# westlake-repl/Adapter4Rec

Measured on NVIDIA B200. Metric: train user-sequences/s (SASRec + BERT-base LoRA r=8 adapter-tuning step: fwd+bwd+allreduce+Adam), higher is better.
Workload: dtype bf16

## Files before the change

adapter4rec_b200/csrc/a4r_common.cuh:

```cuda
#pragma once
#include <cuda.h>
#include <cuda_bf16.h>
#include <cuda_runtime.h>
#include <stdint.h>
#include <stdio.h>

#include "../../include/adapter4rec.h"

int a4r_set_error(int code, const char* fmt, ...);

#define A4R_CHECK_ARG(cond, ...)                                   \
  do {                                                              \
    if (!(cond)) return a4r_set_error(A4R_EINVAL, __VA_ARGS__);     \
  } while (0)

#define A4R_CUDA_OK(expr)                                                                  \
  do {                                                                                      \
    cudaError_t _e = (expr);                                                                \
    if (_e != cudaSuccess)                                                                  \
      return a4r_set_error(A4R_ECUDA, "%s failed: %s (%s:%d)", #expr, cudaGetErrorString(_e), \
                           __FILE__, __LINE__);                                             \
  } while (0)

#define A4R_LAUNCH_OK()                                                                   \
  do {                                                                                     \
    cudaError_t _e = cudaGetLastError();                                                   \
    if (_e != cudaSuccess)                                                                 \
      return a4r_set_error(A4R_ECUDA, "kernel launch failed: %s (%s:%d)",                  \
                           cudaGetErrorString(_e), __FILE__, __LINE__);                    \
  } while (0)

int a4r_num_sms();
void a4r_count_launch(int n);

int a4r_make_tmap_bf16(CUtensorMap* m, const void* base, int64_t rows, int64_t cols, int64_t ld, int box_rows);

static inline bool a4r_aligned16(const void* p) { return (reinterpret_cast<uintptr_t>(p) & 15u) == 0; }

#ifdef __CUDACC__

#define A4R_DEVICE __device__ __forceinline__

A4R_DEVICE uint32_t smem_u32(const void* p) { return static_cast<uint32_t>(__cvta_generic_to_shared(p)); }

A4R_DEVICE float warp_sum(float v) {
#pragma unroll
  for (int o = 16; o > 0; o >>= 1) v += __shfl_xor_sync(0xffffffffu, v, o);
  return v;
}
A4R_DEVICE float warp_max(float v) {
#pragma unroll
  for (int o = 16; o > 0; o >>= 1) v = fmaxf(v, __shfl_xor_sync(0xffffffffu, v, o));
  return v;
}

A4R_DEVICE float gelu_erf(float x) { return 0.5f * x * (1.0f + erff(x * 0.70710678118654752440f)); }
A4R_DEVICE float gelu_erf_grad(float x) {
  const float cdf = 0.5f * (1.0f + erff(x * 0.70710678118654752440f));
  const float pdf = 0.39894228040143267794f * __expf(-0.5f * x * x);
  return cdf + x * pdf;
}

A4R_DEVICE float ex2_approx(float x) {
  float r;
  asm("ex2.approx.ftz.f32 %0, %1;" : "=f"(r) : "f"(x));
  return r;
}
A4R_DEVICE float tanh_approx(float x) {
  float r;
  asm("tanh.approx.f32 %0, %1;" : "=f"(r) : "f"(x));
  return r;
}
constexpr float kGeluC0 = 0.797507884f, kGeluC1 = 0.0370056460f, kGeluC2 = -3.51516783e-4f;
A4R_DEVICE float gelu_cdf(float x) {
  const float x2 = fminf(x * x, 64.0f);
  const float u = x * fmaf(fmaf(x2, kGeluC2, kGeluC1), x2, kGeluC0);
  return fmaf(0.5f, tanh_approx(u), 0.5f);
}
A4R_DEVICE float gelu_fast(float x) { return x * gelu_cdf(x); }
A4R_DEVICE float gelu_grad_fast(float x) {
  const float e = ex2_approx(-0.72134752044448170368f * x * x);
  return fmaf(x * 0.39894228040143267794f, e, gelu_cdf(x));
}
A4R_DEVICE float2 splat2(float c) { return make_float2(c, c); }
A4R_DEVICE float2 gelu_cdf2(float2 x) {
  float2 x2 = __fmul2_rn(x, x);
  x2 = make_float2(fminf(x2.x, 64.0f), fminf(x2.y, 64.0f));
  float2 q = __ffma2_rn(x2, splat2(kGeluC2), splat2(kGeluC1));
// ... 368 lines not shown
```

adapter4rec_b200/csrc/api.cu:

```cuda
#include <stdarg.h>
#include <atomic>

#include "a4r_common.cuh"

namespace {
thread_local char g_err[512] = {0};
std::atomic<int64_t> g_launches{0};
}

int a4r_set_error(int code, const char* fmt, ...) {
  va_list ap;
  va_start(ap, fmt);
  vsnprintf(g_err, sizeof(g_err), fmt, ap);
  va_end(ap);
  return code;
}

void a4r_count_launch(int n) { g_launches.fetch_add(n, std::memory_order_relaxed); }

int a4r_num_sms() {
  static int sms = 0;
  if (sms == 0) {
    int dev = 0;
    if (cudaGetDevice(&dev) != cudaSuccess) return 148;
    if (cudaDeviceGetAttribute(&sms, cudaDevAttrMultiProcessorCount, dev) != cudaSuccess || sms <= 0) sms = 148;
  }
  return sms;
}

namespace {
typedef CUresult (*PFN_encodeTiled)(CUtensorMap*, CUtensorMapDataType, cuuint32_t, void*, const cuuint64_t*,
                                    const cuuint64_t*, const cuuint32_t*, const cuuint32_t*, CUtensorMapInterleave,
                                    CUtensorMapSwizzle, CUtensorMapL2promotion, CUtensorMapFloatOOBfill);
PFN_encodeTiled encode_fn() {
  static PFN_encodeTiled fn = nullptr;
  if (fn == nullptr) {
    void* p = nullptr;
    cudaDriverEntryPointQueryResult q;
    if (cudaGetDriverEntryPoint("cuTensorMapEncodeTiled", &p, cudaEnableDefault, &q) == cudaSuccess &&
        q == cudaDriverEntryPointSuccess)
      fn = reinterpret_cast<PFN_encodeTiled>(p);
  }
  return fn;
}
}

int a4r_make_tmap_bf16(CUtensorMap* m, const void* base, int64_t rows, int64_t cols, int64_t ld, int box_rows) {
  PFN_encodeTiled fn = encode_fn();
  if (fn == nullptr) return a4r_set_error(A4R_ECUDA, "cuTensorMapEncodeTiled entry point not found");
  cuuint64_t dims[2] = {static_cast<cuuint64_t>(cols), static_cast<cuuint64_t>(rows)};
  cuuint64_t strides[1] = {static_cast<cuuint64_t>(ld) * 2};
  cuuint32_t box[2] = {64u, static_cast<cuuint32_t>(box_rows)};
  cuuint32_t estr[2] = {1, 1};
  CUresult r = fn(m, CU_TENSOR_MAP_DATA_TYPE_BFLOAT16, 2, const_cast<void*>(base), dims, strides, box, estr,
                  CU_TENSOR_MAP_INTERLEAVE_NONE, CU_TENSOR_MAP_SWIZZLE_128B, CU_TENSOR_MAP_L2_PROMOTION_L2_256B,
                  CU_TENSOR_MAP_FLOAT_OOB_FILL_NONE);
  if (r != CUDA_SUCCESS)
    return a4r_set_error(A4R_ECUDA, "cuTensorMapEncodeTiled failed (%d) rows=%lld cols=%lld ld=%lld", (int)r,
                         (long long)rows, (long long)cols, (long long)ld);
  return A4R_OK;
}

extern "C" int a4r_version(void) { return 100;  }

extern "C" const char* a4r_last_error_string(void) { return g_err; }

extern "C" int64_t a4r_launch_count(void) { return g_launches.load(std::memory_order_relaxed); }

extern "C" int a4r_device_check(void) {
  static int cached_dev = -1;
  static int cached_rc = A4R_OK;
  int dev = 0;
  cudaError_t e = cudaGetDevice(&dev);
  if (e != cudaSuccess) return a4r_set_error(A4R_ECUDA, "cudaGetDevice failed: %s", cudaGetErrorString(e));
  if (dev == cached_dev) {
    if (cached_rc != A4R_OK) a4r_set_error(cached_rc, "device %d is not compute capability 10.x (sm_100a only)", dev);
    return cached_rc;
  }
  int major = 0;
  e = cudaDeviceGetAttribute(&major, cudaDevAttrComputeCapabilityMajor, dev);
  if (e != cudaSuccess) return a4r_set_error(A4R_ECUDA, "cudaDeviceGetAttribute failed: %s", cudaGetErrorString(e));
  cached_dev = dev;
  cached_rc = (major == 10) ? A4R_OK : A4R_EARCH;
  if (cached_rc != A4R_OK)
    return a4r_set_error(A4R_EARCH, "device %d has compute capability %d.x; this library is sm_100a only", dev, major);
  return A4R_OK;
}
```

adapter4rec_b200/functional.py:

```python
import torch

from . import ops

BF16 = torch.bfloat16


PARAM_EPOCH = [0]


def bump_param_epoch():
    PARAM_EPOCH[0] += 1


class WeightCache:

    def __init__(self):
        self.key = None
        self.master = None
        self.w = None
        self.wt = None

    def get(self, weight, need_t=False):
        key = (weight.data_ptr(), weight._version, weight.device, PARAM_EPOCH[0] if weight.requires_grad else -1)
        if key != self.key:
# ... 355 lines not shown
    first = torch.full((uh.numel(),), N, dtype=torch.int64, device=rows.device)
    first.scatter_reduce_(0, inverse, torch.arange(N, device=rows.device), reduce="amin")
    uniq = rows[first]
    if not bool((uniq[inverse] == rows).all()):
        uniq, inverse, counts = torch.unique(rows, dim=0, return_inverse=True, return_counts=True)
    return uniq, inverse, counts


LORA_PAD = 64


class QKVFunction(torch.autograd.Function):

    @staticmethod
    def forward(ctx, x, cache, *params):
        ctx.with_skip = len(params) > 0 and isinstance(params[-1], str) and params[-1] == "skip"
        if ctx.with_skip:
            params = params[:-1]
        ctx.set_materialize_grads(False)
        assert len(params) % 4 == 0
        n = len(params) // 4
        H = params[0].shape[0]
        K = params[0].shape[1]
        dev = x.device
        frozen_w = not any(p is not None and p.requires_grad for p in [params[4 * j] for j in range(n)])
        key = tuple((p.data_ptr(), p._version) for p in [params[4 * j] for j in range(n)]) + (PARAM_EPOCH[0] if not frozen_w else -1,)
        if cache.get("key") != key or not frozen_w:
            cache["key"] = key
            cache["w"] = torch.cat([params[i].detach().to(BF16) for i in range(0, 4 * n, 4)], 0).contiguous()
            cache["wt"] = None
        w = cache["w"]
        small = [params[4 * j + i] for j in range(n) for i in (1, 2, 3)]
        skey = (PARAM_EPOCH[0],) + tuple(None if p is None else (p.data_ptr(), p._version) for p in small)
        reuse = cache.get("small_key") == skey
        if reuse:
            bias = cache["bias"]
        else:
            zero_h = cache.get("zero_h")
            if zero_h is None or zero_h.device != dev or zero_h.numel() != H:
                zero_h = cache["zero_h"] = torch.zeros(H, dtype=torch.float32, device=dev)
            bias = torch.cat([zero_h if params[4 * j + 1] is None else params[4 * j + 1].detach().float() for j in range(n)])
            cache["small_key"], cache["bias"] = skey, bias
        slots, off = [], 0
        for j in range(n):
            A = params[4 * j + 2]
            if A is not None:
                r = A.shape[0]
                slots.append((j, off, r))
                off += r
        assert off <= LORA_PAD, "sum of LoRA ranks of one fused projection must be <= 64"
        T = a_cat = b_ext = None
        if slots:
            ctx.ones_col = off < LORA_PAD
            if reuse and "a_cat" in cache:
                a_cat, b_ext, t_bias = cache["a_cat"], cache["b_ext"], cache["t_bias"]
            else:
                st = cache.get("lora_stage")
                if st is None or st[0].device != dev or st[0].shape != (LORA_PAD, K) or st[1].shape != (n * H, LORA_PAD):
                    st = cache["lora_stage"] = (torch.zeros((LORA_PAD, K), dtype=torch.float32, device=dev),
                                                torch.zeros((n * H, LORA_PAD), dtype=torch.float32, device=dev))
                    cache["lora_slots"] = None
                if cache.get("lora_slots") != slots:
                    st[0].zero_()
                    st[1].zero_()
                    cache["lora_slots"] = list(slots)
                for j, o, r in slots:
                    st[0][o:o + r].copy_(params[4 * j + 2].detach())
                    torch.mul(params[4 * j + 3].detach(), 1.0 / r, out=st[1][j * H:(j + 1) * H, o:o + r])
                a_cat, a_cat_t = ops.cast_transpose(st[0], True, True)
                b_ext, b_ext_t = ops.cast_transpose(st[1], True, True)
                tb = cache.get("t_bias_const")
                if tb is None or tb[0] != ctx.ones_col or tb[1].device != dev:
                    t_bias = torch.zeros(LORA_PAD, dtype=torch.float32, device=dev)
                    if ctx.ones_col:
                        t_bias[LORA_PAD - 1] = 1.0
                    tb = cache["t_bias_const"] = (ctx.ones_col, t_bias)
                t_bias = tb[1]
                cache["a_cat"], cache["b_ext"], cache["t_bias"] = a_cat, b_ext, t_bias
                cache["a_cat_t"], cache["b_ext_t"] = a_cat_t, b_ext_t
            T = ops.gemm(x, a_cat, bias=t_bias)
            qkv = ops.gemm(x, w, bias=bias, a2=T, b2=b_ext)
        else:
            qkv = ops.gemm(x, w, bias=bias)
        ctx.cache, ctx.slots, ctx.H, ctx.n = cache, slots, H, n
        if not slots:
            ctx.ones_col = False
        ctx.n_params = len(params)
        ctx.param_needs = [p is not None and p.requires_grad for p in params]
        need_x = any(ctx.param_needs[4 * j + 2] for j in range(n)) or any(ctx.param_needs[4 * j] for j in range(n))
        ctx.save_for_backward(x if need_x else None, T, a_cat, b_ext)
        if ctx.with_skip:
            return qkv, x
        return qkv

    @staticmethod
    def backward(ctx, dqkv, dskip=None):
        x, T, a_cat, b_ext = ctx.saved_tensors
        H, cache, n = ctx.H, ctx.cache, ctx.n
        tail = (None,) if ctx.with_skip else ()
        if dqkv is None:
            return (dskip, None) + (None,) * ctx.n_params + tail
        dqkv = dqkv.contiguous()
        if dskip is not None:
            dskip = dskip.contiguous()
        if cache.get("wt") is None:
            cache["wt"] = cache["w"].t().contiguous()
        grads = [None] * ctx.n_params
        dT = None
        if ctx.slots:
            if cache.get("b_ext") is b_ext and cache.get("b_ext_t") is not None:
                b_ext_t, a_cat_t = cache["b_ext_t"], cache["a_cat_t"]
            else:
                b_ext_t, a_cat_t = b_ext.t().contiguous(), a_cat.t().contiguous()
                if cache.get("b_ext") is b_ext:
                    cache["b_ext_t"], cache["a_cat_t"] = b_ext_t, a_cat_t
            lj = [j for j, _, _ in ctx.slots]
            if n == 3 and len(lj) == 2:
                (ja, jb) = lj
                dT = ops.gemm(dqkv[:, ja * H:(ja + 1) * H], b_ext_t[:, ja * H:(ja + 1) * H],
                              a2=dqkv[:, jb * H:(jb + 1) * H], b2=b_ext_t[:, jb * H:(jb + 1) * H])
            elif n == 3 and len(lj) == 1:
                dT = ops.gemm(dqkv[:, lj[0] * H:(lj[0] + 1) * H], b_ext_t[:, lj[0] * H:(lj[0] + 1) * H])
            else:
                dT = ops.gemm(dqkv, b_ext_t)
            dx = ops.gemm(dqkv, cache["wt"], a2=dT, b2=a_cat_t, residual=dskip) if ctx.needs_input_grad[0] else None
        else:
            dx = ops.gemm(dqkv, cache["wt"], residual=dskip) if ctx.needs_input_grad[0] else None
        fused = bool(ctx.slots) and ctx.ones_col
        if fused:
            want_g1 = any(ctx.param_needs[4 * j + 1] for j in range(n)) or any(ctx.param_needs[4 * j + 3] for j, _, _ in ctx.slots)
            want_g2 = any(ctx.param_needs[4 * j + 2] for j, _, _ in ctx.slots)
            g1_rows = [ctx.param_needs[4 * j + 1] or any(jj == j and ctx.param_needs[4 * j + 3] for jj, _, _ in ctx.slots)
                       for j in range(n)]
            g1 = [None] * n
            if want_g1:
                if all(g1_rows):
                    full = ops.wgrad(dqkv, T)
                    g1 = [full[j * H:(j + 1) * H] for j in range(n)]
                else:
                    g1 = [ops.wgrad(dqkv[:, j * H:(j + 1) * H], T) if g1_rows[j] else None for j in range(n)]
            g2 = ops.wgrad(dT, x) if want_g2 else None
        for j in range(n):
            dq = dqkv[:, j * H:(j + 1) * H]
            if ctx.param_needs[4 * j]:
                grads[4 * j] = ops.wgrad(dq, x)
            if ctx.param_needs[4 * j + 1]:
                grads[4 * j + 1] = g1[j][:, LORA_PAD - 1].contiguous() if fused else ops.colsum(dq)
        for j, o, r in ctx.slots:
            dq = dqkv[:, j * H:(j + 1) * H]
            if ctx.param_needs[4 * j + 3]:
                grads[4 * j + 3] = (g1[j][:, o:o + r] * (1.0 / r)) if fused else \
                    _pad_cols_wgrad(dq, T, o, r, 1.0 / r, transpose=False)
            if ctx.param_needs[4 * j + 2]:
                grads[4 * j + 2] = g2[o:o + r].contiguous() if fused else _pad_cols_wgrad(dT, x, o, r, 1.0, transpose=True)
        return (dx, None) + tuple(grads) + tail


def _pad_cols_wgrad(a, b, off, r, alpha, transpose):
    lo = (off // 8) * 8
    hi = ((off + r + 7) // 8) * 8
    if transpose:
        full = ops.wgrad(a[:, lo:hi], b, alpha=alpha)
        return full[off - lo:off - lo + r].contiguous()
    full = ops.wgrad(a, b[:, lo:hi], alpha=alpha)
    return full[:, off - lo:off - lo + r].contiguous()


class EmbedLNFunction(torch.autograd.Function):

    @staticmethod
    def forward(ctx, ids, L, tables, gamma, beta, eps, roberta_pad_id, prompt, word_pad_idx, *params):
        word, pos, typ = tables
        need_prompt = prompt is not None and prompt.requires_grad
        need_tab = [p is not None and p.requires_grad for p in params] + [False] * (5 - len(params))
        need = need_prompt or any(need_tab)
        p16 = None if prompt is None else prompt.detach().to(BF16).contiguous()
        out, z, mean, rstd = ops.embed_ln_fwd(ids, L, word, pos, typ, gamma, beta, eps, roberta_pad_id=roberta_pad_id,
                                              prompt=p16, want_z=need)
        ctx.L, ctx.need_prompt, ctx.need_tab, ctx.roberta_pad_id, ctx.word_pad_idx = L, need_prompt, need_tab, roberta_pad_id, word_pad_idx
        ctx.n_prompt = 0 if prompt is None else prompt.shape[0]
        ctx.shapes = [None if p is None else tuple(p.shape) for p in params]
        if need:
            ctx.save_for_backward(z, mean, rstd, gamma, ids)
        return out

    @staticmethod
    def backward(ctx, dout):
        z, mean, rstd, gamma, ids = ctx.saved_tensors
        need_word, need_pos, need_typ, need_g, need_b = ctx.need_tab
        dg = db = None
        if need_g or need_b:
            dg, db = torch.empty_like(gamma), torch.empty_like(gamma)
        dz = ops.layernorm_bwd(dout.contiguous(), z, mean, rstd, gamma, dgamma=dg, dbeta=db)
        H = dz.shape[1]
        L, n = ctx.L, ctx.n_prompt
        dp = None
        if ctx.need_prompt:
            dp = ops.colsum(dz.view(-1, L * H), width=n * H).view(n, H)
        grads = [None] * len(ctx.shapes)
        tok = ids[:, :L]
        if need_word:
            idx = tok.clone()
            if n > 0:
                idx[:, :n] = -1
# ... 195 lines not shown
```

adapter4rec_b200/lib.py:

```python
import ctypes
import os
from ctypes import POINTER, Structure, c_char_p, c_float, c_int32, c_int64, c_size_t, c_void_p

HERE = os.path.dirname(os.path.abspath(__file__))
LIB_PATH = os.path.join(HERE, "libadapter4rec_sm100.so")

A4R_OK, A4R_EINVAL, A4R_ECUDA, A4R_EARCH, A4R_EWORKSPACE = 0, -1, -2, -3, -4
EPI_LINEAR, EPI_GELU, EPI_RELU, EPI_DGELU, EPI_DRELU = 0, 1, 2, 3, 4


class GemmArgs(Structure):
    _fields_ = [
        ("A", c_void_p), ("lda", c_int64), ("B", c_void_p), ("ldb", c_int64),
        ("A2", c_void_p), ("lda2", c_int64), ("B2", c_void_p), ("ldb2", c_int64), ("K2", c_int64),
        ("C", c_void_p), ("ldc", c_int64), ("aux", c_void_p), ("ldaux", c_int64),
        ("residual", c_void_p), ("ldr", c_int64), ("residual2", c_void_p), ("ldr2", c_int64),
        ("bias", c_void_p), ("M", c_int64), ("N", c_int64), ("K", c_int64),
        ("alpha", c_float), ("epilogue", c_int32), ("out_f32", c_int32), ("block_n", c_int32),
        ("dropout_p", c_float), ("dropout_seed", ctypes.c_uint64), ("dropout_offset", ctypes.c_uint64),
        ("dropout_after_residual", c_int32),
    ]


class AttnArgs(Structure):
# ... 29 lines not shown
class AdapterArgs(Structure):
    _fields_ = [
        ("h", c_void_p), ("ldh", c_int64), ("input", c_void_p), ("ldi", c_int64),
        ("w_down", c_void_p), ("b_down", c_void_p), ("w_up", c_void_p), ("b_up", c_void_p),
        ("gamma", c_void_p), ("beta", c_void_p), ("out", c_void_p), ("z_out", c_void_p),
        ("mean", c_void_p), ("rstd", c_void_p), ("s_out", c_void_p), ("u_out", c_void_p),
        ("M", c_int64), ("H", c_int64), ("r", c_int64), ("act", c_int32), ("tail", c_int32), ("eps", c_float),
        ("lds", c_int64), ("impl", c_int32),
    ]


class InbatchCeArgs(Structure):
    _fields_ = [
        ("prec", c_void_p), ("cand", c_void_p), ("ld_cand", c_int64), ("item_ids", c_void_p), ("log_mask", c_void_p),
        ("cand_bias", c_void_p), ("lse", c_void_p), ("loss", c_void_p), ("count", c_void_p),
        ("B", c_int64), ("S", c_int64), ("D", c_int64), ("masked_logit", c_float),
    ]


PROTOTYPES = {
    "a4r_version": (c_int32, []),
    "a4r_last_error_string": (c_char_p, []),
    "a4r_device_check": (c_int32, []),
    "a4r_launch_count": (c_int64, []),
    "a4r_gemm_bf16_tn": (c_int32, [POINTER(GemmArgs), c_void_p]),
    "a4r_attn_small_fwd": (c_int32, [POINTER(AttnArgs), c_void_p]),
    "a4r_attn_small_bwd": (c_int32, [POINTER(AttnArgs), c_void_p]),
    "a4r_attn_mid_fwd": (c_int32, [POINTER(AttnArgs), c_void_p]),
    "a4r_attn_mid_bwd": (c_int32, [POINTER(AttnArgs), c_void_p]),
    "a4r_layernorm_fwd": (c_int32, [c_void_p, c_void_p, c_int64, c_void_p, c_void_p, c_float, c_void_p, c_void_p,
                                    c_void_p, c_void_p, c_int64, c_int64, c_void_p]),
    "a4r_layernorm_bwd_workspace_bytes": (c_size_t, [c_int64]),
    "a4r_layernorm_bwd": (c_int32, [c_void_p, c_void_p, c_void_p, c_void_p, c_void_p, c_void_p, c_void_p, c_void_p,
                                    c_int32, c_void_p, c_size_t, c_int64, c_int64, c_void_p, c_float, ctypes.c_uint64,
                                    ctypes.c_uint64, c_void_p]),
    "a4r_layernorm_bwd_add": (c_int32, [c_void_p, c_void_p, c_void_p, c_void_p, c_void_p, c_void_p, c_void_p, c_int64, c_int64,
                                        c_void_p]),
    "a4r_adapter_ln_supported": (c_int32, [c_int64, c_int64]),
    "a4r_adapter_ln_fwd": (c_int32, [POINTER(AdapterArgs), c_void_p]),
    "a4r_embed_ln_fwd": (c_int32, [POINTER(EmbedArgs), c_void_p]),
    "a4r_act_bwd": (c_int32, [c_void_p, c_void_p, c_void_p, c_int64, c_int32, c_void_p]),
    "a4r_act_fwd": (c_int32, [c_void_p, c_void_p, c_int64, c_int32, c_void_p]),
    "a4r_scatter_add_rows": (c_int32, [c_void_p, c_int64, c_void_p, c_void_p, c_int64, c_int64, c_int64, c_int64, c_void_p]),
    "a4r_cast_transpose_f32_bf16": (c_int32, [c_void_p, c_int64, c_void_p, c_void_p, c_int64, c_int64, c_void_p]),
    "a4r_dropout": (c_int32, [c_void_p, c_void_p, c_void_p, c_int64, c_float, ctypes.c_uint64, ctypes.c_uint64, c_void_p]),
    "a4r_colsum_workspace_bytes": (c_size_t, [c_int64]),
    "a4r_colsum": (c_int32, [c_void_p, c_int64, c_int64, c_int64, c_void_p, c_int32, c_void_p, c_size_t, c_void_p]),
    "a4r_wgrad_workspace_bytes": (c_size_t, [c_int64, c_int64, c_int64]),
    "a4r_wgrad_bf16": (c_int32, [c_void_p, c_int64, c_void_p, c_int64, c_void_p, c_int64, c_int64, c_int64, c_int64,
                                 c_float, c_int32, c_void_p, c_size_t, c_void_p]),
    "a4r_wgrad_tc_workspace_bytes": (c_size_t, [c_int64, c_int64, c_int64]),
    "a4r_wgrad_tc_bf16": (c_int32, [c_void_p, c_int64, c_void_p, c_int64, c_void_p, c_int64, c_int64, c_int64, c_int64,
                                    c_float, c_int32, c_void_p, c_size_t, c_void_p]),
    "a4r_bce_workspace_bytes": (c_size_t, []),
    "a4r_bce_loss_fwd": (c_int32, [POINTER(BceArgs), c_void_p, c_size_t, c_void_p]),
    "a4r_bce_loss_bwd": (c_int32, [POINTER(BceArgs), c_void_p, c_void_p, c_void_p, c_void_p]),
    "a4r_inbatch_ce_workspace_bytes": (c_size_t, [c_int64, c_int64]),
    "a4r_inbatch_ce_fwd": (c_int32, [POINTER(InbatchCeArgs), c_void_p, c_size_t, c_void_p]),
    "a4r_inbatch_ce_bwd": (c_int32, [POINTER(InbatchCeArgs), c_void_p, c_void_p, c_void_p, c_int64, c_void_p]),
    "a4r_adam_step": (c_int32, [c_void_p, c_void_p, c_void_p, c_void_p, c_int64, c_float, c_float, c_float, c_float,
                                c_float, c_int64, c_float, c_void_p]),
    "a4r_adam_step_dev": (c_int32, [c_void_p, c_void_p, c_void_p, c_void_p, c_int64, c_float, c_float, c_float, c_float,
                                    c_float, c_void_p, c_float, c_void_p]),
    "a4r_patchify": (c_int32, [c_void_p, c_void_p, c_int64, c_int64, c_int64, c_int64, c_void_p]),
    "a4r_vit_assemble": (c_int32, [c_void_p, c_void_p, c_void_p, c_void_p, c_void_p, c_int64, c_int64, c_int64, c_int64,
                                   c_void_p]),
    "a4r_gather_rows": (c_int32, [c_void_p, c_void_p, c_void_p, c_int64, c_int64, c_void_p]),
    "a4r_sample_train_batch": (c_int32, [c_void_p, c_void_p, c_void_p, c_void_p, c_void_p, c_void_p, c_void_p, c_int64,
                                         c_int64, c_int64, c_int64, ctypes.c_uint64, ctypes.c_uint64, c_void_p]),
    "a4r_score_topk_partials": (c_int32, [c_int64, c_int64]),
    "a4r_score_topk": (c_int32, [c_void_p, c_int64, c_void_p, c_int64, c_int64, c_int64, c_int64, c_int64, c_void_p,
                                 c_int64, c_int32, c_void_p, c_void_p, c_void_p]),
    "a4r_topk_merge": (c_int32, [c_void_p, c_void_p, c_int32, c_int64, c_int32, c_void_p, c_void_p, c_void_p, c_void_p,
                                 c_void_p, c_void_p]),
}

_lib = None


def get_lib():
    global _lib
    if _lib is None:
        if not os.path.exists(LIB_PATH):
            raise RuntimeError(
                "adapter4rec_b200: %s is missing — build it with __graft_entry__.build() "
                "(there is no CPU or PyTorch fallback for this path)" % LIB_PATH)
        lib = ctypes.CDLL(LIB_PATH)
        for name, (restype, argtypes) in PROTOTYPES.items():
            fn = getattr(lib, name)
            fn.restype = restype
            fn.argtypes = argtypes
        _lib = lib
    return _lib


def check(rc, what):
    if rc != A4R_OK:
        msg = get_lib().a4r_last_error_string()
        raise RuntimeError("%s failed (code %d): %s" % (what, rc, msg.decode() if msg else ""))


def launch_count():
    return int(get_lib().a4r_launch_count())
```

adapter4rec_b200/ops.py:

```python
import ctypes

import torch

from . import lib as _l
from .lib import EPI_DGELU, EPI_DRELU, EPI_GELU, EPI_LINEAR, EPI_RELU

BF16 = torch.bfloat16
F32_MIN = -3.4028234663852886e38


def _stream():
    return ctypes.c_void_p(torch.cuda.current_stream().cuda_stream)


def _p(t):
    return None if t is None else ctypes.c_void_p(t.data_ptr())


def _rows2d(t, name):
    if t.dim() != 2 or t.stride(1) != 1:
        raise ValueError("%s must be 2-D with unit column stride, got shape %s stride %s" % (name, tuple(t.shape), t.stride()))
    return t.stride(0) if t.shape[0] > 1 else max(t.stride(0), t.shape[1])


# ... 255 lines not shown
    M = x.shape[0]
    width = x.shape[1] if width is None else width
    if out is None and width == x.shape[1] and width <= 128 and x.is_contiguous() and M >= 4096:
        f = 16
        while f > 1 and M % f:
            f //= 2
        if f > 1:
            return colsum(x.view(M // f, f * width)).view(f, width).sum(0)
    if out is None:
        out = torch.empty(width, dtype=torch.float32, device=x.device)
        accumulate = False
    wsb = _l.get_lib().a4r_colsum_workspace_bytes(width)
    ws = workspace(wsb, x.device)
    _l.check(_l.get_lib().a4r_colsum(_p(x), _rows2d(x, "x"), M, width, _p(out), int(accumulate), _p(ws), wsb, _stream()),
             "a4r_colsum")
    return out


def wgrad_mma_sync(a, b, alpha=1.0, out=None, accumulate=False, n=None, k=None):
    assert a.dtype == BF16 and b.dtype == BF16 and a.shape[0] == b.shape[0]
    M = a.shape[0]
    N = a.shape[1] if n is None else n
    K = b.shape[1] if k is None else k
    if out is None:
        out = torch.empty((N, K), dtype=torch.float32, device=a.device)
        accumulate = False
    assert out.dtype == torch.float32 and tuple(out.shape) == (N, K) and out.stride(1) == 1
    wsb = _l.get_lib().a4r_wgrad_workspace_bytes(M, N, K)
    ws = workspace(wsb, a.device)
    _l.check(_l.get_lib().a4r_wgrad_bf16(_p(a), _rows2d(a, "a"), _p(b), _rows2d(b, "b"), _p(out), out.stride(0), M, N, K,
                                         float(alpha), int(accumulate), _p(ws), wsb, _stream()), "a4r_wgrad_bf16")
    return out


def wgrad_tc(a, b, alpha=1.0, out=None, accumulate=False, n=None, k=None):
    assert a.dtype == BF16 and b.dtype == BF16 and a.shape[0] == b.shape[0]
    M = a.shape[0]
    N = a.shape[1] if n is None else n
    K = b.shape[1] if k is None else k
    if out is None:
        out = torch.empty((N, K), dtype=torch.float32, device=a.device)
        accumulate = False
    assert out.dtype == torch.float32 and tuple(out.shape) == (N, K) and out.stride(1) == 1
    wsb = _l.get_lib().a4r_wgrad_tc_workspace_bytes(M, N, K)
    ws = workspace(wsb, a.device)
    _l.check(_l.get_lib().a4r_wgrad_tc_bf16(_p(a), _rows2d(a, "a"), _p(b), _rows2d(b, "b"), _p(out), out.stride(0), M, N, K,
                                            float(alpha), int(accumulate), _p(ws), wsb, _stream()), "a4r_wgrad_tc_bf16")
    return out


wgrad = wgrad_tc


def _bce_args(prec, emb, log_mask, pos, neg, loss, count, cpc):
    B, S, D = prec.shape
    assert prec.dtype == BF16 and emb.dtype == BF16 and prec.is_contiguous() and emb.is_contiguous()
    assert emb.numel() == B * (S + 1) * 2 * D
    a = _l.BceArgs()
    a.prec, a.emb, a.log_mask = _p(prec), _p(emb), _p(log_mask)
    a.pos_score, a.neg_score, a.loss, a.count = _p(pos), _p(neg), _p(loss), _p(count)
    a.B, a.S, a.D, a.cpc = B, S, D, int(cpc)
    return a


def bce_loss_fwd(prec, emb, log_mask, cpc=False):
    B, S, _ = prec.shape
    dev = prec.device
    pos = torch.empty((B, S), dtype=torch.float32, device=dev)
    neg = torch.empty((B, S), dtype=torch.float32, device=dev)
    loss = torch.empty(1, dtype=torch.float32, device=dev)
    count = torch.empty(1, dtype=torch.float32, device=dev)
    if log_mask is not None:
        assert log_mask.dtype == torch.float32 and log_mask.is_contiguous() and tuple(log_mask.shape) == (B, S)
    a = _bce_args(prec, emb, log_mask, pos, neg, loss, count, cpc)
    wsb = _l.get_lib().a4r_bce_workspace_bytes()
    ws = workspace(wsb, dev)
    _l.check(_l.get_lib().a4r_bce_loss_fwd(ctypes.byref(a), _p(ws), wsb, _stream()), "a4r_bce_loss_fwd")
    return loss, count, pos, neg


def bce_loss_bwd(prec, emb, log_mask, pos, neg, count, grad_out=None, cpc=False):
    d_prec = torch.empty_like(prec)
    d_emb = torch.empty_like(emb)
    loss = torch.empty(1, dtype=torch.float32, device=prec.device)
    a = _bce_args(prec, emb, log_mask, pos, neg, loss, count, cpc)
    if grad_out is not None:
        assert grad_out.dtype == torch.float32 and grad_out.numel() == 1
    _l.check(_l.get_lib().a4r_bce_loss_bwd(ctypes.byref(a), _p(grad_out), _p(d_prec), _p(d_emb), _stream()),
             "a4r_bce_loss_bwd")
    return d_prec, d_emb


def adapter_ln_supported(H, r):
    return bool(_l.get_lib().a4r_adapter_ln_supported(int(H), int(r)))


def adapter_ln_fwd(h, inp, w_down, b_down, w_up, b_up, gamma=None, beta=None, eps=0.0, act="relu", tail=0, save=False,
                   impl=0):
    assert h.dtype == BF16 and h.dim() == 2 and w_down.dtype == BF16 and w_up.dtype == BF16
    assert w_down.is_contiguous() and w_up.is_contiguous()
    M, H = h.shape
    r = w_down.shape[0]
    assert tuple(w_down.shape) == (r, H) and tuple(w_up.shape) == (H, r)
    for t in (b_down, b_up) + ((gamma, beta) if tail == 0 else ()):
        assert t.dtype == torch.float32 and t.is_contiguous()
    dev = h.device
# ... 177 lines not shown
```

include/adapter4rec.h:

```cpp
#ifndef ADAPTER4REC_H_
#define ADAPTER4REC_H_

#include <stddef.h>
#include <stdint.h>

#ifdef __cplusplus
extern "C" {
#endif

#define A4R_OK 0
#define A4R_EINVAL (-1)
#define A4R_ECUDA (-2)
#define A4R_EARCH (-3)
#define A4R_EWORKSPACE (-4)

typedef void* a4r_stream_t;

#define A4R_API __attribute__((visibility("default")))

A4R_API int a4r_version(void);
A4R_API const char* a4r_last_error_string(void);
A4R_API int a4r_device_check(void);
A4R_API int64_t a4r_launch_count(void);

// ... 102 lines not shown

typedef struct a4r_embed_args {
  const int64_t* ids;
  int64_t ld_ids;
  const void* word_emb;
  const void* pos_emb;
  const void* type_emb;
  const void* prompt;
  const float* gamma;
  const float* beta;
  void* out;
  void* z_out;
  float* mean_out;
  float* rstd_out;
  int64_t N, L, H;
  int64_t pos_offset;
  int64_t roberta_pad_id;
  int64_t n_prompt;
  float eps;
} a4r_embed_args;
A4R_API int a4r_embed_ln_fwd(const a4r_embed_args* args, a4r_stream_t stream);

A4R_API int a4r_patchify(const float* images, void* out, int64_t N, int64_t C, int64_t R, int64_t ps, a4r_stream_t stream);
A4R_API int a4r_vit_assemble(const void* patch_emb, const void* cls, const void* pos, const void* prompt, void* out,
                             int64_t N, int64_t P, int64_t T, int64_t H, a4r_stream_t stream);

A4R_API int a4r_scatter_add_rows(const void* src, int64_t ld, const int64_t* idx, float* dst, int64_t R, int64_t H,
                                 int64_t V, int64_t skip_idx, a4r_stream_t stream);

A4R_API int a4r_act_bwd(const void* dy, const void* u, void* out, int64_t n, int32_t kind, a4r_stream_t stream);
A4R_API int a4r_act_fwd(const void* u, void* out, int64_t n, int32_t kind, a4r_stream_t stream);

A4R_API int a4r_cast_transpose_f32_bf16(const float* src, int64_t ld_src, void* dst, void* dst_t, int64_t rows, int64_t cols,
                                        a4r_stream_t stream);

A4R_API int a4r_dropout(const void* x, const void* res, void* out, int64_t n, float p, uint64_t seed, uint64_t offset,
                        a4r_stream_t stream);
#define A4R_SEED_INDIRECT (1ull << 63)

A4R_API size_t a4r_colsum_workspace_bytes(int64_t width);
A4R_API int a4r_colsum(const void* x, int64_t ld, int64_t M, int64_t width, float* out, int32_t accumulate,
               void* workspace, size_t workspace_bytes, a4r_stream_t stream);

A4R_API size_t a4r_wgrad_workspace_bytes(int64_t M, int64_t N, int64_t K);
A4R_API int a4r_wgrad_bf16(const void* A, int64_t lda, const void* B, int64_t ldb, float* dW, int64_t ldw, int64_t M,
                   int64_t N, int64_t K, float alpha, int32_t accumulate, void* workspace, size_t workspace_bytes,
                   a4r_stream_t stream);

A4R_API size_t a4r_wgrad_tc_workspace_bytes(int64_t M, int64_t N, int64_t K);
A4R_API int a4r_wgrad_tc_bf16(const void* A, int64_t lda, const void* B, int64_t ldb, float* dW, int64_t ldw, int64_t M,
                              int64_t N, int64_t K, float alpha, int32_t accumulate, void* workspace,
                              size_t workspace_bytes, a4r_stream_t stream);

typedef struct a4r_bce_args {
  const void* prec;
  const void* emb;
  const float* log_mask;
  float* pos_score;
  float* neg_score;
  float* loss;
  float* count;
  int64_t B, S, D;
  int32_t cpc;
} a4r_bce_args;
A4R_API size_t a4r_bce_workspace_bytes(void);
A4R_API int a4r_bce_loss_fwd(const a4r_bce_args* args, void* workspace, size_t workspace_bytes, a4r_stream_t stream);
A4R_API int a4r_bce_loss_bwd(const a4r_bce_args* args, const float* grad_out, void* d_prec, void* d_emb,
                     a4r_stream_t stream);

typedef struct a4r_inbatch_ce_args {
  const void* prec;
  const void* cand;
  int64_t ld_cand;
  const int64_t* item_ids;
  const float* log_mask;
  const float* cand_bias;
  float* lse;
  float* loss;
  float* count;
  int64_t B, S, D;
  float masked_logit;
} a4r_inbatch_ce_args;
A4R_API size_t a4r_inbatch_ce_workspace_bytes(int64_t B, int64_t S);
A4R_API int a4r_inbatch_ce_fwd(const a4r_inbatch_ce_args* args, void* workspace, size_t workspace_bytes, a4r_stream_t stream);
A4R_API int a4r_inbatch_ce_bwd(const a4r_inbatch_ce_args* args, const float* grad_out, void* d_prec, void* d_cand,
                               int64_t ld_dcand, a4r_stream_t stream);

A4R_API int a4r_adam_step(float* p, const float* g, float* m, float* v, int64_t n, float lr, float beta1, float beta2,
                  float eps, float weight_decay, int64_t step, float grad_scale, a4r_stream_t stream);
A4R_API int a4r_adam_step_dev(float* p, const float* g, float* m, float* v, int64_t n, float lr, float beta1, float beta2,
                              float eps, float weight_decay, const float* bias_corr, float grad_scale, a4r_stream_t stream);

A4R_API int a4r_gather_rows(const void* table, const int64_t* ids, void* out, int64_t rows, int64_t D,
                            a4r_stream_t stream);

A4R_API int a4r_sample_train_batch(const int64_t* seqs, const int64_t* item_content, const int64_t* neg_in, int64_t* out,
                                   float* log_mask, int64_t* neg_out, int32_t* fail_flag, int64_t B, int64_t S1, int64_t W,
                                   int64_t item_num, uint64_t seed, uint64_t offset, a4r_stream_t stream);

A4R_API int a4r_score_topk_partials(int64_t U, int64_t I);
A4R_API int a4r_score_topk(const void* users, int64_t ld_users, const void* items, int64_t ld_items, int64_t U, int64_t I,
                           int64_t d, int64_t id_base, const int32_t* history, int64_t hist_len, int32_t k,
                           float* out_scores, int32_t* out_ids, a4r_stream_t stream);

A4R_API int a4r_topk_merge(const float* in_scores, const int32_t* in_ids, int32_t P, int64_t U, int32_t k,
                           float* out_scores, int32_t* out_ids, const int32_t* target, float* hit, float* ndcg,
// ... 7 lines not shown
```

Measured before the change: 1974.

## Fuse LoRA q/v backward dT GEMM and dB/db wgrad into one tcgen05 kernel

```diff
diff --git a/adapter4rec_b200/csrc/a4r_common.cuh b/adapter4rec_b200/csrc/a4r_common.cuh
--- a/adapter4rec_b200/csrc/a4r_common.cuh
+++ b/adapter4rec_b200/csrc/a4r_common.cuh
@@ -34,6 +34,7 @@
 void a4r_count_launch(int n);
 
 int a4r_make_tmap_bf16(CUtensorMap* m, const void* base, int64_t rows, int64_t cols, int64_t ld, int box_rows);
+int a4r_make_tmap_bf16_sw64(CUtensorMap* m, const void* base, int64_t rows, int64_t cols, int64_t ld, int box_rows);
 
 static inline bool a4r_aligned16(const void* p) { return (reinterpret_cast<uintptr_t>(p) & 15u) == 0; }
 
diff --git a/adapter4rec_b200/csrc/api.cu b/adapter4rec_b200/csrc/api.cu
--- a/adapter4rec_b200/csrc/api.cu
+++ b/adapter4rec_b200/csrc/api.cu
@@ -61,6 +61,22 @@
   return A4R_OK;
 }
 
+int a4r_make_tmap_bf16_sw64(CUtensorMap* m, const void* base, int64_t rows, int64_t cols, int64_t ld, int box_rows) {
+  PFN_encodeTiled fn = encode_fn();
+  if (fn == nullptr) return a4r_set_error(A4R_ECUDA, "cuTensorMapEncodeTiled entry point not found");
+  cuuint64_t dims[2] = {static_cast<cuuint64_t>(cols), static_cast<cuuint64_t>(rows)};
+  cuuint64_t strides[1] = {static_cast<cuuint64_t>(ld) * 2};
+  cuuint32_t box[2] = {32u, static_cast<cuuint32_t>(box_rows)};
+  cuuint32_t estr[2] = {1, 1};
+  CUresult r = fn(m, CU_TENSOR_MAP_DATA_TYPE_BFLOAT16, 2, const_cast<void*>(base), dims, strides, box, estr,
+                  CU_TENSOR_MAP_INTERLEAVE_NONE, CU_TENSOR_MAP_SWIZZLE_64B, CU_TENSOR_MAP_L2_PROMOTION_NONE,
+                  CU_TENSOR_MAP_FLOAT_OOB_FILL_NONE);
+  if (r != CUDA_SUCCESS)
+    return a4r_set_error(A4R_ECUDA, "cuTensorMapEncodeTiled (64B swizzle) failed (%d) rows=%lld cols=%lld ld=%lld", (int)r,
+                         (long long)rows, (long long)cols, (long long)ld);
+  return A4R_OK;
+}
+
 extern "C" int a4r_version(void) { return 100;  }
 
 extern "C" const char* a4r_last_error_string(void) { return g_err; }
diff --git a/adapter4rec_b200/csrc/lora_bwd_sm100.cu b/adapter4rec_b200/csrc/lora_bwd_sm100.cu
--- /dev/null
+++ b/adapter4rec_b200/csrc/lora_bwd_sm100.cu
@@ -0,0 +1,320 @@
+#include "a4r_common.cuh"
+
+namespace {
+
+constexpr int BT = 128;
+constexpr int BOX = BT * 64 * 2;
+constexpr int BBOX = 64 * 64 * 2;
+constexpr int kStage = 2 * BOX + 2 * BBOX;
+constexpr int kStages = 4;
+constexpr int TBOX = BT * 32 * 2;
+constexpr int GW = 32;
+constexpr int kSmem = kStages * kStage + 2 * TBOX + 1024 + 256;
+constexpr uint32_t kTmemCols = 512;
+constexpr int kMaxH = (512 - 128) / GW * 128 / 2;
+
+struct LParams {
+  __nv_bfloat16* dT;
+  float* partial;
+  int M, H;
+  int col_a, col_b;
+  int nchunks;
+};
+
+A4R_DEVICE uint64_t desc_mn_sw128_pair(uint32_t smem_addr) {
+  uint64_t d = 0;
+  d |= static_cast<uint64_t>((smem_addr & 0x3FFFFu) >> 4);
+  d |= static_cast<uint64_t>(BOX >> 4) << 16;
+  d |= static_cast<uint64_t>(1024 >> 4) << 32;
+  d |= static_cast<uint64_t>(1) << 46;
+  d |= static_cast<uint64_t>(2) << 61;
+  return d;
+}
+A4R_DEVICE uint64_t desc_mn_sw64(uint32_t smem_addr) {
+  uint64_t d = 0;
+  d |= static_cast<uint64_t>((smem_addr & 0x3FFFFu) >> 4);
+  d |= static_cast<uint64_t>(1) << 16;
+  d |= static_cast<uint64_t>(512 >> 4) << 32;
+  d |= static_cast<uint64_t>(1) << 46;
+  d |= static_cast<uint64_t>(4) << 61;
+  return d;
+}
+
+__global__ void __launch_bounds__(256, 1)
+lora_qv_bwd_kernel(const __grid_constant__ CUtensorMap tmD, const __grid_constant__ CUtensorMap tmB,
+                   const __grid_constant__ CUtensorMap tmT, const LParams p) {
+  extern __shared__ uint8_t smem_raw[];
+  uint8_t* smem = reinterpret_cast<uint8_t*>((reinterpret_cast<uintptr_t>(smem_raw) + 1023) & ~uintptr_t(1023));
+  uint8_t* tbuf = smem + kStages * kStage;
+  uint64_t* full_bar = reinterpret_cast<uint64_t*>(tbuf + 2 * TBOX);
+  uint64_t* empty_bar = full_bar + kStages;
+  uint64_t* tfull_bar = empty_bar + kStages;
+  uint64_t* tempty_bar = tfull_bar + 2;
+  uint64_t* dfull_bar = tempty_bar + 2;
+  uint64_t* dempty_bar = dfull_bar + 2;
+  uint64_t* gfull_bar = dempty_bar + 2;
+  uint32_t* tmem_slot = reinterpret_cast<uint32_t*>(gfull_bar + 1);
+
+  const int warp = __shfl_sync(0xffffffffu, threadIdx.x >> 5, 0);
+  const int lane = threadIdx.x & 31;
+  const int c_begin = static_cast<int>(static_cast<int64_t>(blockIdx.x) * p.nchunks / gridDim.x);
+  const int c_end = static_cast<int>(static_cast<int64_t>(blockIdx.x + 1) * p.nchunks / gridDim.x);
+  const int nloc = c_end - c_begin;
+  const int kpairs = p.H / 128;
+  const int npairs = 2 * kpairs;
+
+  if (warp == 0 && lane == 0) {
+    tma_prefetch_desc(&tmD);
+    tma_prefetch_desc(&tmB);
+    tma_prefetch_desc(&tmT);
+  }
+  if (warp == 1 && lane == 0) {
+    for (int s = 0; s < kStages; ++s) {
+      mbar_init(&full_bar[s], 1);
+      mbar_init(&empty_bar[s], 1);
+    }
+    for (int s = 0; s < 2; ++s) {
+      mbar_init(&tfull_bar[s], 1);
+      mbar_init(&tempty_bar[s], 1);
+      mbar_init(&dfull_bar[s], 1);
+      mbar_init(&dempty_bar[s], 4);
+    }
+    mbar_init(gfull_bar, 1);
+    mbar_fence_init();
+  }
+  if (warp == 2) {
+    tmem_alloc(tmem_slot, kTmemCols);
+    tmem_relinquish();
+  }
+  tc_fence_before();
+  __syncthreads();
+  tc_fence_after();
+  const uint32_t tmem_base = *tmem_slot;
+
+  if (warp == 0) {
+    int stage = 0;
+    uint32_t phase = 0;
+    for (int li = 0; li < nloc; ++li) {
+      const int t0 = (c_begin + li) * BT;
+      const int tb = li & 1;
+      mbar_wait(&tempty_bar[tb], ((li >> 1) & 1) ^ 1);
+      __syncwarp();
+      tma_load_2d_elect(&tmT, tbuf + tb * TBOX, &tfull_bar[tb], 0, t0, TBOX);
+      for (int pp = 0; pp < npairs; ++pp) {
+        const int col = pp < kpairs ? p.col_a + pp * 128 : p.col_b + (pp - kpairs) * 128;
+        mbar_wait(&empty_bar[stage], phase ^ 1);
+        __syncwarp();
+        uint8_t* sa = smem + stage * kStage;
+        mbar_expect_tx_elect(&full_bar[stage], kStage);
+        tma_load_2d_elect_noarm(&tmD, sa, &full_bar[stage], col, t0);
+        tma_load_2d_elect_noarm(&tmD, sa + BOX, &full_bar[stage], col + 64, t0);
+        tma_load_2d_elect_noarm(&tmB, sa + 2 * BOX, &full_bar[stage], col, 0);
+        tma_load_2d_elect_noarm(&tmB, sa + 2 * BOX + BBOX, &full_bar[stage], col + 64, 0);
+        if (++stage == kStages) {
+          stage = 0;
+          phase ^= 1;
+        }
+      }
+    }
+  } else if (warp == 1) {
+    constexpr uint32_t idesc_dt = umma_idesc_bf16(BT, 64);
+    constexpr uint32_t idesc_g = umma_idesc_bf16(128, GW) | (1u << 15) | (1u << 16);
+    int stage = 0;
+    uint32_t phase = 0;
+    for (int li = 0; li < nloc; ++li) {
+      const int as = li & 1;
+      mbar_wait(&dempty_bar[as], ((li >> 1) & 1) ^ 1);
+      __syncwarp();
+      mbar_wait(&tfull_bar[as], (li >> 1) & 1);
+      __syncwarp();
+      tc_fence_after();
+      const uint32_t tmem_d = tmem_base + static_cast<uint32_t>(as * 64);
+      const uint64_t tdesc = desc_mn_sw64(smem_u32(tbuf + as * TBOX));
+      for (int pp = 0; pp < npairs; ++pp) {
+        mbar_wait(&full_bar[stage], phase);
+        __syncwarp();
+        tc_fence_after();
+        const uint32_t sa = smem_u32(smem + stage * kStage);
+#pragma unroll
+        for (int h = 0; h < 2; ++h) {
+          const uint64_t adesc = umma_desc_k_sw128(sa + h * BOX);
+          const uint64_t bdesc = umma_desc_k_sw128(sa + 2 * BOX + h * BBOX);
+#pragma unroll
+          for (int k = 0; k < 4; ++k)
+            umma_bf16_ss_elect(tmem_d, adesc + static_cast<uint64_t>(k * 2), bdesc + static_cast<uint64_t>(k * 2), idesc_dt,
+                               (pp | h | k) != 0 ? 1u : 0u);
+        }
+        const uint64_t gdesc = desc_mn_sw128_pair(sa);
+        const uint32_t tmem_g = tmem_base + 128u + static_cast<uint32_t>(pp * GW);
+#pragma unroll
+        for (int k = 0; k < BT / 16; ++k)
+          umma_bf16_ss_elect(tmem_g, gdesc + static_cast<uint64_t>(k * 128), tdesc + static_cast<uint64_t>(k * 64), idesc_g,
+                             (li | k) != 0 ? 1u : 0u);
+        umma_commit_elect(&empty_bar[stage]);
+        if (++stage == kStages) {
+          stage = 0;
+          phase ^= 1;
+        }
+      }
+      umma_commit_elect(&dfull_bar[as]);
+      umma_commit_elect(&tempty_bar[as]);
+    }
+    umma_commit_elect(gfull_bar);
+  } else if (warp >= 4) {
+    const int quad = warp & 3;
+    const uint32_t lane_addr = static_cast<uint32_t>(quad * 32) << 16;
+    for (int li = 0; li < nloc; ++li) {
+      const int as = li & 1;
+      const int row = (c_begin + li) * BT + quad * 32 + lane;
+      mbar_wait(&dfull_bar[as], (li >> 1) & 1);
+      tc_fence_after();
+      uint32_t a0[32], a1[32];
+      tmem_ld_32x32b_x32(tmem_base + lane_addr + static_cast<uint32_t>(as * 64), a0);
+      tmem_ld_32x32b_x32(tmem_base + lane_addr + static_cast<uint32_t>(as * 64 + 32), a1);
+      tmem_ld_wait();
+      tc_fence_before();
+      __syncwarp();
+      if (lane == 0) mbar_arrive(&dempty_bar[as]);
+      if (row < p.M) {
+        __nv_bfloat16* dst = p.dT + static_cast<int64_t>(row) * 64;
+        uint32_t w[8];
+#pragma unroll
+        for (int j = 0; j < 2; ++j) {
+#pragma unroll
+          for (int i = 0; i < 8; ++i) w[i] = pack_bf16x2(__uint_as_float(a0[16 * j + 2 * i]), __uint_as_float(a0[16 * j + 2 * i + 1]));
+          st_na_v8(dst + 16 * j, w);
+        }
+#pragma unroll
+        for (int j = 0; j < 2; ++j) {
+#pragma unroll
+          for (int i = 0; i < 8; ++i) w[i] = pack_bf16x2(__uint_as_float(a1[16 * j + 2 * i]), __uint_as_float(a1[16 * j + 2 * i + 1]));
+          st_na_v8(dst + 32 + 16 * j, w);
+        }
+      }
+    }
+    mbar_wait(gfull_bar, 0);
+    tc_fence_after();
+    float* dst = p.partial + (static_cast<int64_t>(blockIdx.x) * 2 * p.H + quad * 32 + lane) * GW;
+#pragma unroll 1
+    for (int g = 0; g < npairs; ++g) {
+      uint32_t acc[32];
+      tmem_ld_32x32b_x32(tmem_base + lane_addr + 128u + static_cast<uint32_t>(g * GW), acc);
+      tmem_ld_wait();
+#pragma unroll
+      for (int j = 0; j < 8; ++j)
+        st_na_v4(dst + static_cast<int64_t>(g) * 128 * GW + 4 * j, make_uint4(acc[4 * j], acc[4 * j + 1], acc[4 * j + 2], acc[4 * j + 3]));
+    }
+    tc_fence_before();
+  }
+  tc_fence_before();
+  __syncthreads();
+  tc_fence_after();
+  if (warp == 2) tmem_dealloc(tmem_base, kTmemCols);
+}
+
+struct RParams {
+  const float* partial;
+  int splits, H;
+  int off[2], r[2];
+  int ones;
+  float* dB[2];
+  float* db[2];
+};
+
+__global__ void lora_qv_reduce_kernel(const RParams p) {
+  const int i = blockIdx.x * blockDim.x + threadIdx.x;
+  if (i >= 2 * p.H * GW) return;
+  const int row2 = i / GW, c = i % GW;
+  const bool seg = row2 >= p.H;
+  const int row = seg ? row2 - p.H : row2;
+  const int off = seg ? p.off[1] : p.off[0], r = seg ? p.r[1] : p.r[0];
+  float* dB = seg ? p.dB[1] : p.dB[0];
+  float* db = seg ? p.db[1] : p.db[0];
+  const bool want_B = dB != nullptr && c >= off && c < off + r;
+  const bool want_b = db != nullptr && c == p.ones;
+  if (!want_B && !want_b) return;
+  float s = 0.f;
+#pragma unroll 8
+  for (int sp = 0; sp < p.splits; ++sp) s += p.partial[(static_cast<int64_t>(sp) * 2 * p.H + row2) * GW + c];
+  if (want_B) dB[static_cast<int64_t>(row) * r + (c - off)] = s * (1.0f / static_cast<float>(r));
+  if (want_b) db[row] = s;
+}
+
+int plan_grid(int64_t M) {
+  const int64_t nchunks = (M + BT - 1) / BT;
+  const int sms = a4r_num_sms();
+  return static_cast<int>(nchunks < sms ? nchunks : sms);
+}
+
+}
+
+extern "C" size_t a4r_lora_qv_bwd_workspace_bytes(int64_t M, int64_t H) {
+  return static_cast<size_t>(plan_grid(M)) * 2 * static_cast<size_t>(H) * GW * sizeof(float);
+}
+
+extern "C" int a4r_lora_qv_bwd(const void* dqkv, int64_t ld, int64_t col_a, int64_t col_b, const void* b_ext_t, int64_t ldb,
+                               const void* T, int64_t ldt, void* dT, int64_t M, int64_t H, int32_t off_a, int32_t r_a,
+                               int32_t off_b, int32_t r_b, int32_t ones_col, float* dB_a, float* db_a, float* dB_b,
+                               float* db_b, void* workspace, size_t workspace_bytes, a4r_stream_t stream_) {
+  A4R_CHECK_ARG(M >= 0 && M < (1ll << 31), "lora_qv_bwd: M out of range");
+  A4R_CHECK_ARG(H >= 128 && H <= kMaxH && H % 128 == 0, "lora_qv_bwd: H must be a multiple of 128 in [128, %d]", kMaxH);
+  A4R_CHECK_ARG(col_a >= 0 && col_b >= 0 && col_a % 8 == 0 && col_b % 8 == 0 && col_a + H <= ld && col_b + H <= ld &&
+                    ld % 8 == 0 && ld < (1ll << 24),
+                "lora_qv_bwd: bad dqkv columns / leading dimension");
+  A4R_CHECK_ARG(ldb >= col_a + H && ldb >= col_b + H && ldb % 8 == 0, "lora_qv_bwd: bad B_ext^T leading dimension");
+  A4R_CHECK_ARG(ldt >= 32 && ldt % 8 == 0, "lora_qv_bwd: T needs >= 32 columns, ldt % 8 == 0");
+  A4R_CHECK_ARG(r_a > 0 && r_b > 0 && off_a >= 0 && off_b >= 0 && off_a + r_a <= GW && off_b + r_b <= GW && ones_col >= 0 &&
+                    ones_col < GW,
+                "lora_qv_bwd: LoRA slots and the ones column must lie in T columns [0, 32)");
+  A4R_CHECK_ARG(M == 0 || (dqkv && b_ext_t && T && dT), "lora_qv_bwd: NULL pointer");
+  A4R_CHECK_ARG(a4r_aligned16(dqkv) && a4r_aligned16(b_ext_t) && a4r_aligned16(T) &&
+                    (reinterpret_cast<uintptr_t>(dT) & 31u) == 0,
+                "lora_qv_bwd: dqkv, B_ext^T and T must be 16B aligned, dT 32B aligned");
+  const size_t need = a4r_lora_qv_bwd_workspace_bytes(M, H);
+  if (need > 0 && (workspace == nullptr || workspace_bytes < need))
+    return a4r_set_error(A4R_EWORKSPACE, "lora_qv_bwd: workspace too small (%zu < %zu)", workspace_bytes, need);
+  A4R_CHECK_ARG(a4r_aligned16(workspace), "lora_qv_bwd: workspace must be 16B aligned");
+  int rc = a4r_device_check();
+  if (rc != A4R_OK) return rc;
+  cudaStream_t stream = static_cast<cudaStream_t>(stream_);
+  const int grid = plan_grid(M);
+  if (grid > 0) {
+    CUtensorMap tmD, tmB, tmT;
+    const int64_t cols = (col_a > col_b ? col_a : col_b) + H;
+    if ((rc = a4r_make_tmap_bf16(&tmD, dqkv, M, cols, ld, BT)) != A4R_OK) return rc;
+    if ((rc = a4r_make_tmap_bf16(&tmB, b_ext_t, 64, cols, ldb, 64)) != A4R_OK) return rc;
+    if ((rc = a4r_make_tmap_bf16_sw64(&tmT, T, M, GW, ldt, BT)) != A4R_OK) return rc;
+    LParams p;
+    p.dT = static_cast<__nv_bfloat16*>(dT);
+    p.partial = static_cast<float*>(workspace);
+    p.M = static_cast<int>(M);
+    p.H = static_cast<int>(H);
+    p.col_a = static_cast<int>(col_a);
+    p.col_b = static_cast<int>(col_b);
+    p.nchunks = static_cast<int>((M + BT - 1) / BT);
+    static bool attr_done = false;
+    if (!attr_done) {
+      A4R_CUDA_OK(cudaFuncSetAttribute(lora_qv_bwd_kernel, cudaFuncAttributeMaxDynamicSharedMemorySize, kSmem));
+      attr_done = true;
+    }
+    lora_qv_bwd_kernel<<<grid, 256, kSmem, stream>>>(tmD, tmB, tmT, p);
+    A4R_LAUNCH_OK();
+    a4r_count_launch(1);
+  }
+  if (dB_a || db_a || dB_b || db_b) {
+    RParams r;
+    r.partial = static_cast<const float*>(workspace);
+    r.splits = grid;
+    r.H = static_cast<int>(H);
+    r.off[0] = off_a, r.off[1] = off_b;
+    r.r[0] = r_a, r.r[1] = r_b;
+    r.ones = ones_col;
+    r.dB[0] = dB_a, r.dB[1] = dB_b;
+    r.db[0] = db_a, r.db[1] = db_b;
+    const int total = 2 * static_cast<int>(H) * GW;
+    lora_qv_reduce_kernel<<<(total + 255) / 256, 256, 0, stream>>>(r);
+    A4R_LAUNCH_OK();
+    a4r_count_launch(1);
+  }
+  return A4R_OK;
+}
diff --git a/adapter4rec_b200/functional.py b/adapter4rec_b200/functional.py
--- a/adapter4rec_b200/functional.py
+++ b/adapter4rec_b200/functional.py
@@ -431,6 +431,7 @@
         T = a_cat = b_ext = None
         if slots:
             ctx.ones_col = off < LORA_PAD
+            ctx.ones_idx = off
             if reuse and "a_cat" in cache:
                 a_cat, b_ext, t_bias = cache["a_cat"], cache["b_ext"], cache["t_bias"]
             else:
@@ -449,11 +450,11 @@
                 a_cat, a_cat_t = ops.cast_transpose(st[0], True, True)
                 b_ext, b_ext_t = ops.cast_transpose(st[1], True, True)
                 tb = cache.get("t_bias_const")
-                if tb is None or tb[0] != ctx.ones_col or tb[1].device != dev:
+                if tb is None or tb[0] != off or tb[1].device != dev:
                     t_bias = torch.zeros(LORA_PAD, dtype=torch.float32, device=dev)
                     if ctx.ones_col:
-                        t_bias[LORA_PAD - 1] = 1.0
-                    tb = cache["t_bias_const"] = (ctx.ones_col, t_bias)
+                        t_bias[off] = 1.0
+                    tb = cache["t_bias_const"] = (off, t_bias)
                 t_bias = tb[1]
                 cache["a_cat"], cache["b_ext"], cache["t_bias"] = a_cat, b_ext, t_bias
                 cache["a_cat_t"], cache["b_ext_t"] = a_cat_t, b_ext_t
@@ -486,6 +487,7 @@
             cache["wt"] = cache["w"].t().contiguous()
         grads = [None] * ctx.n_params
         dT = None
+        qv = None
         if ctx.slots:
             if cache.get("b_ext") is b_ext and cache.get("b_ext_t") is not None:
                 b_ext_t, a_cat_t = cache["b_ext_t"], cache["a_cat_t"]
@@ -494,7 +496,15 @@
                 if cache.get("b_ext") is b_ext:
                     cache["b_ext_t"], cache["a_cat_t"] = b_ext_t, a_cat_t
             lj = [j for j, _, _ in ctx.slots]
-            if n == 3 and len(lj) == 2:
+            qv_slots = [(o, r) for _, o, r in ctx.slots]
+            if n == 3 and len(lj) == 2 and ctx.ones_col and ops.lora_qv_bwd_supported(H, qv_slots, ctx.ones_idx) \
+                    and not any(ctx.param_needs[4 * j + 1] for j in range(n) if j not in lj):
+                ja, jb = lj
+                dT, ga, gb = ops.lora_qv_bwd(dqkv, ja * H, jb * H, H, b_ext_t, T, qv_slots, ctx.ones_idx,
+                                             want_B=[ctx.param_needs[4 * ja + 3], ctx.param_needs[4 * jb + 3]],
+                                             want_b=[ctx.param_needs[4 * ja + 1], ctx.param_needs[4 * jb + 1]])
+                qv = {ja: ga, jb: gb}
+            elif n == 3 and len(lj) == 2:
                 (ja, jb) = lj
                 dT = ops.gemm(dqkv[:, ja * H:(ja + 1) * H], b_ext_t[:, ja * H:(ja + 1) * H],
                               a2=dqkv[:, jb * H:(jb + 1) * H], b2=b_ext_t[:, jb * H:(jb + 1) * H])
@@ -512,7 +522,7 @@
             g1_rows = [ctx.param_needs[4 * j + 1] or any(jj == j and ctx.param_needs[4 * j + 3] for jj, _, _ in ctx.slots)
                        for j in range(n)]
             g1 = [None] * n
-            if want_g1:
+            if want_g1 and qv is None:
                 if all(g1_rows):
                     full = ops.wgrad(dqkv, T)
                     g1 = [full[j * H:(j + 1) * H] for j in range(n)]
@@ -524,11 +534,14 @@
             if ctx.param_needs[4 * j]:
                 grads[4 * j] = ops.wgrad(dq, x)
             if ctx.param_needs[4 * j + 1]:
-                grads[4 * j + 1] = g1[j][:, LORA_PAD - 1].contiguous() if fused else ops.colsum(dq)
+                if qv is not None:
+                    grads[4 * j + 1] = qv[j][1]
+                else:
+                    grads[4 * j + 1] = g1[j][:, ctx.ones_idx].contiguous() if fused else ops.colsum(dq)
         for j, o, r in ctx.slots:
             dq = dqkv[:, j * H:(j + 1) * H]
             if ctx.param_needs[4 * j + 3]:
-                grads[4 * j + 3] = (g1[j][:, o:o + r] * (1.0 / r)) if fused else \
+                grads[4 * j + 3] = qv[j][0] if qv is not None else (g1[j][:, o:o + r] * (1.0 / r)) if fused else \
                     _pad_cols_wgrad(dq, T, o, r, 1.0 / r, transpose=False)
             if ctx.param_needs[4 * j + 2]:
                 grads[4 * j + 2] = g2[o:o + r].contiguous() if fused else _pad_cols_wgrad(dT, x, o, r, 1.0, transpose=True)
diff --git a/adapter4rec_b200/lib.py b/adapter4rec_b200/lib.py
--- a/adapter4rec_b200/lib.py
+++ b/adapter4rec_b200/lib.py
@@ -105,6 +105,10 @@
     "a4r_wgrad_tc_workspace_bytes": (c_size_t, [c_int64, c_int64, c_int64]),
     "a4r_wgrad_tc_bf16": (c_int32, [c_void_p, c_int64, c_void_p, c_int64, c_void_p, c_int64, c_int64, c_int64, c_int64,
                                     c_float, c_int32, c_void_p, c_size_t, c_void_p]),
+    "a4r_lora_qv_bwd_workspace_bytes": (c_size_t, [c_int64, c_int64]),
+    "a4r_lora_qv_bwd": (c_int32, [c_void_p, c_int64, c_int64, c_int64, c_void_p, c_int64, c_void_p, c_int64, c_void_p,
+                                  c_int64, c_int64, c_int32, c_int32, c_int32, c_int32, c_int32, c_void_p, c_void_p,
+                                  c_void_p, c_void_p, c_void_p, c_size_t, c_void_p]),
     "a4r_bce_workspace_bytes": (c_size_t, []),
     "a4r_bce_loss_fwd": (c_int32, [POINTER(BceArgs), c_void_p, c_size_t, c_void_p]),
     "a4r_bce_loss_bwd": (c_int32, [POINTER(BceArgs), c_void_p, c_void_p, c_void_p, c_void_p]),
diff --git a/adapter4rec_b200/ops.py b/adapter4rec_b200/ops.py
--- a/adapter4rec_b200/ops.py
+++ b/adapter4rec_b200/ops.py
@@ -331,6 +331,26 @@
 wgrad = wgrad_tc
 
 
+def lora_qv_bwd_supported(H, slots, ones_col):
+    return H % 128 == 0 and 128 <= H <= 768 and len(slots) == 2 and all(o + r <= 32 for o, r in slots) and ones_col < 32
+
+
+def lora_qv_bwd(dqkv, col_a, col_b, H, b_ext_t, T, slots, ones_col, want_B, want_b):
+    assert dqkv.dtype == BF16 and b_ext_t.dtype == BF16 and T.dtype == BF16
+    M = dqkv.shape[0]
+    dev = dqkv.device
+    dT = torch.empty((M, 64), dtype=BF16, device=dev)
+    dB = [torch.empty((H, r), dtype=torch.float32, device=dev) if w else None for (_, r), w in zip(slots, want_B)]
+    db = [torch.empty(H, dtype=torch.float32, device=dev) if w else None for w in want_b]
+    wsb = _l.get_lib().a4r_lora_qv_bwd_workspace_bytes(M, H)
+    ws = workspace(wsb, dev)
+    (oa, ra), (ob, rb) = slots
+    _l.check(_l.get_lib().a4r_lora_qv_bwd(_p(dqkv), _rows2d(dqkv, "dqkv"), col_a, col_b, _p(b_ext_t), _rows2d(b_ext_t, "b_ext_t"),
+                                          _p(T), _rows2d(T, "T"), _p(dT), M, H, oa, ra, ob, rb, ones_col, _p(dB[0]), _p(db[0]),
+                                          _p(dB[1]), _p(db[1]), _p(ws), wsb, _stream()), "a4r_lora_qv_bwd")
+    return dT, (dB[0], db[0]), (dB[1], db[1])
+
+
 def _bce_args(prec, emb, log_mask, pos, neg, loss, count, cpc):
     B, S, D = prec.shape
     assert prec.dtype == BF16 and emb.dtype == BF16 and prec.is_contiguous() and emb.is_contiguous()
diff --git a/include/adapter4rec.h b/include/adapter4rec.h
--- a/include/adapter4rec.h
+++ b/include/adapter4rec.h
@@ -178,6 +178,12 @@
                               int64_t N, int64_t K, float alpha, int32_t accumulate, void* workspace,
                               size_t workspace_bytes, a4r_stream_t stream);
 
+A4R_API size_t a4r_lora_qv_bwd_workspace_bytes(int64_t M, int64_t H);
+A4R_API int a4r_lora_qv_bwd(const void* dqkv, int64_t ld, int64_t col_a, int64_t col_b, const void* b_ext_t, int64_t ldb,
+                            const void* T, int64_t ldt, void* dT, int64_t M, int64_t H, int32_t off_a, int32_t r_a,
+                            int32_t off_b, int32_t r_b, int32_t ones_col, float* dB_a, float* db_a, float* dB_b,
+                            float* db_b, void* workspace, size_t workspace_bytes, a4r_stream_t stream);
+
 typedef struct a4r_bce_args {
   const void* prec;
   const void* emb;
```

After: 2001, median of 6. +1.3%, better.
